# thu-wangz17/HermNet

Hardware: AMD Instinct MI355X
Metric: atom-steps/sec (energy+forces) on 10k-atom 3-element cell; HBM GB/s vs roofline (higher is better)
Workload: dtype f32; 1 GPU; configs[1]: 10000-atom 3-element fcc alloy (Al/Ni/Cu), HVNet rc=5.0 hidden=128 num_rbf=128 layers=5, E=431340 directed edges, energy+forces per step; config=c2, atoms_total=10000, atoms_owned_rank0=10000, halo_atoms_rank0=0, edges_rank0=431340, tuned_gemm_table=False, gemm_tuning_in_warmup=False, parallelism=1 GPU

## Files before the change

### hermnet_amd/csrc/message_bwd_cl.hip

```cpp
#include <hip/hip_runtime.h>
#include <stdint.h>
#include <type_traits>
#include "../../include/hermnet_hip.h"
#include "hermnet_math.h"
#include "message_bwd_cl.h"

namespace {

typedef float hn_f2 __attribute__((ext_vector_type(2)));
typedef unsigned hn_u2 __attribute__((ext_vector_type(2)));
typedef __attribute__((address_space(4))) const float hn_cfloat;
typedef __attribute__((address_space(4))) const int hn_cint;

constexpr int kRec = HN_EDGE_TABLE_FLOATS;

#ifndef HN_NT_TABLE
#define HN_NT_TABLE 1
#endif
__device__ __forceinline__ float fwd_envelope_val(float u, int kind, int p) {
#pragma clang fp contract(off)
  if (kind != 0 || !(u < 1.0f)) return hn_envelope(u, kind, p).val;
  const float up = hn_powi(u, p - 1) * u;
  const float w = 1.0f - u;
  const float fp = (float)p;
  const float inner = __builtin_fmaf(0.5f * fp * (fp + 1.0f), w, fp);
  const float q = 1.0f + w * inner;
  return __builtin_fmaf(-q, up, 1.0f);
}
__global__ __launch_bounds__(256) void edge_table_kernel(const float4* __restrict__ edge, const int* __restrict__ csc_pos,
                                                         int E, const float* __restrict__ offset, int R, float inv_rc,
                                                         float coeff, int env_kind, int env_p,
                                                         float* __restrict__ table, const int* __restrict__ csc_end,
                                                         float* __restrict__ fwd_taps, int csc_blocks) {
  constexpr int kLd = kRec + 4;
  __shared__ __align__(16) float stage[4][64 * kLd];
  const int lane = threadIdx.x & 63, wave = threadIdx.x >> 6;
  if ((int)blockIdx.x >= csc_blocks) {
    constexpr int kF = HN_FWD_TAPS_FLOATS, kLdF = kF + 4;
    const int e0 = (((int)blockIdx.x - csc_blocks) * 4 + wave) * 64;
    if (e0 >= E) return;
    const float u = edge[min(e0 + lane, E - 1)].w * inv_rc;
    const float env_val = fwd_envelope_val(u, env_kind, env_p);
    const int lo = hn_window_lo(u, R);
    float t[kF];
#pragma unroll
    for (int m = 0; m < HN_TAPS; ++m) {
      int k = lo + m;
      k = k < 0 ? 0 : (k >= R ? R - 1 : k);
      const float diff = u - offset[k];
      t[m] = __expf(coeff * (diff * diff));
    }
    t[12] = env_val;
    t[13] = __int_as_float(lo + HN_PAD);
    t[14] = t[15] = 0.f;
    float* st = stage[wave];
#pragma unroll
    for (int w = 0; w < kF / 4; ++w)
      *reinterpret_cast<float4*>(st + lane * kLdF + 4 * w) = make_float4(t[4 * w], t[4 * w + 1], t[4 * w + 2], t[4 * w + 3]);
    const int nrec = min(64, E - e0);
    float4* out = reinterpret_cast<float4*>(fwd_taps + (size_t)e0 * kF);
#pragma unroll
    for (int j = 0; j < kF / 4; ++j) {
      const int idx = j * 64 + lane, r = idx / (kF / 4), w = idx % (kF / 4);
      if (r < nrec) out[idx] = *reinterpret_cast<const float4*>(st + r * kLdF + 4 * w);
    }
    return;
  }
  const int q0 = (blockIdx.x * 4 + wave) * 64;
  if (q0 >= E) return;
  const int q = q0 + lane;
  const int n_csc = csc_end[0];
  float rec[kRec];
#pragma unroll
  for (int w = 0; w < kRec; ++w) rec[w] = 0.f;
  rec[24] = __int_as_float(HN_PAD);
  rec[25] = __int_as_float(HN_PAD);
  if (q < n_csc) {
    const float4 g = edge[csc_pos[q]];
    const float d_next = edge[csc_pos[min(q + 1, n_csc - 1)]].w;
    const float u = g.w * inv_rc;
    const HnEnv env = hn_envelope(u, env_kind, env_p);
    const int lo = hn_window_lo(u, R);
    const float c0 = inv_rc * env.der, c1 = inv_rc * env.val * 2.0f * coeff;
#pragma unroll
    for (int m = 0; m < HN_TAPS; ++m) {
      int k = lo + m;
      k = k < 0 ? 0 : (k >= R ? R - 1 : k);
      const float diff = u - offset[k];
      const float gm = __expf(coeff * (diff * diff));
      rec[2 * m] = env.val * gm;
      rec[2 * m + 1] = c0 * gm + c1 * (gm * diff);
    }
    rec[24] = __int_as_float(lo + HN_PAD);
    rec[25] = __int_as_float(hn_window_lo(d_next * inv_rc, R) + HN_PAD);
    rec[28] = g.x; rec[29] = g.y; rec[30] = g.z;
    rec[31] = __builtin_amdgcn_rcpf(g.w);
  }
  float* st = stage[wave];
#pragma unroll
  for (int w = 0; w < kRec / 4; ++w)
    *reinterpret_cast<float4*>(st + lane * kLd + 4 * w) = make_float4(rec[4 * w], rec[4 * w + 1], rec[4 * w + 2], rec[4 * w + 3]);
  const int nrec = min(64, E - q0);
  float4* out = reinterpret_cast<float4*>(table + (size_t)q0 * kRec);
#pragma unroll
  for (int j = 0; j < kRec / 4; ++j) {
    const int idx = j * 64 + lane, r = idx / (kRec / 4), w = idx % (kRec / 4);
    if (r < nrec) {
#if HN_NT_TABLE
      typedef float f4v __attribute__((ext_vector_type(4)));
      __builtin_nontemporal_store(*reinterpret_cast<const f4v*>(st + r * kLd + 4 * w), reinterpret_cast<f4v*>(out + idx));
#else
      out[idx] = *reinterpret_cast<const float4*>(st + r * kLd + 4 * w);
#endif
    }
  }
  if (q0 + nrec == E && lane < kRec / 4)
    out[(size_t)nrec * (kRec / 4) + lane] = *reinterpret_cast<const float4*>(st + (nrec - 1) * kLd + 4 * lane);
}

template <int CTRL>
__device__ __forceinline__ float dpp_mov(float v) {
  return __int_as_float(__builtin_amdgcn_update_dpp(0, __float_as_int(v), CTRL, 0xF, 0xF, false));
}

__device__ __forceinline__ float pair_fold(float e0, float e1) {
  const hn_u2 s = __builtin_amdgcn_permlane32_swap(__float_as_uint(e0), __float_as_uint(e1), false, false);
  return __uint_as_float(s[0]) + __uint_as_float(s[1]);
}
__device__ __forceinline__ float quad_total(float u, float w) {
  const hn_u2 s = __builtin_amdgcn_permlane16_swap(__float_as_uint(u), __float_as_uint(w), false, false);
  float v = __uint_as_float(s[0]) + __uint_as_float(s[1]);
  v += dpp_mov<0xB1>(v);
  v += dpp_mov<0x4E>(v);
  v += dpp_mov<0x141>(v);
  v += dpp_mov<0x140>(v);
  return v;
}

typedef float hn_f4 __attribute__((ext_vector_type(4)));
__device__ __forceinline__ void lds_issue4(unsigned addr, hn_f4 (&w)[4]) {
  asm volatile(
      "ds_read_b128 %0, %4\n\t"
      "ds_read_b128 %1, %4 offset:1024\n\t"
      "ds_read_b128 %2, %4 offset:2048\n\t"
      "ds_read_b128 %3, %4 offset:3072"
      : "=&v"(w[0]), "=&v"(w[1]), "=&v"(w[2]), "=&v"(w[3])
      : "v"(addr)
      : "memory");
}
__device__ __forceinline__ void lds_wait_all(hn_f4 (&wa)[4], hn_f4 (&wb)[4], hn_f4 (&wc)[4]) {
  asm volatile("s_waitcnt lgkmcnt(0)"
               : "+v"(wa[0]), "+v"(wa[1]), "+v"(wa[2]), "+v"(wa[3]), "+v"(wb[0]), "+v"(wb[1]), "+v"(wb[2]), "+v"(wb[3]),
                 "+v"(wc[0]), "+v"(wc[1]), "+v"(wc[2]), "+v"(wc[3])
               :: "memory");
}
static_assert(HN_CB * 16 == 1024 && HN_TAPS == 12, "the tap reader hard-codes the 1 KiB row pitch and 3 x 4 taps");

typedef __amdgpu_buffer_rsrc_t hn_rsrc;
__device__ __forceinline__ float buf_load(hn_rsrc r, unsigned voff, unsigned soff) {
  return __uint_as_float(__builtin_amdgcn_raw_buffer_load_b32(r, voff, soff, 0));
}

__device__ __forceinline__ void buf_store(hn_rsrc r, unsigned voff, unsigned soff, float v) {
  __builtin_amdgcn_raw_buffer_store_b32(__float_as_uint(v), r, voff, soff, 0);
}
#ifndef HN_NT_MSG
#define HN_NT_MSG 1
#endif
__device__ __forceinline__ float buf_load_once(hn_rsrc r, unsigned voff, unsigned soff) {
  return __uint_as_float(__builtin_amdgcn_raw_buffer_load_b32(r, voff, soff, HN_NT_MSG ? 2 : 0));
}
__device__ __forceinline__ hn_rsrc row_rsrc(unsigned long long base, unsigned row_offset_elems, int H) {
  return __builtin_amdgcn_make_buffer_rsrc((void*)(base + (unsigned long long)row_offset_elems * 4ull), 0, 3 * H * 4, 0x00020000);
}
__device__ __forceinline__ unsigned long long uniform_addr(const void* p) {
  const unsigned long long v = (unsigned long long)p;
  const unsigned lo = (unsigned)__builtin_amdgcn_readfirstlane((int)(unsigned)v);
  const unsigned hi = (unsigned)__builtin_amdgcn_readfirstlane((int)(unsigned)(v >> 32));
  return ((unsigned long long)hi << 32) | lo;
}

struct EdgeIn {
  float gx1, g0, g1, g2;
};

#ifndef HN_KO_BWD
#define HN_KO_BWD 0
#endif
template <bool HAS_VEC, bool WIN, bool NEED_GXH>
__device__ __forceinline__ void message_scatter_bwd_cl_body(const HnBwdClArgs& a) {
  static_assert(NEED_GXH || !HAS_VEC, "rows with a vec part always hand gradients down");
  extern __shared__ __align__(16) float4 tile[];
  const int tile_rows = WIN ? a.win_rows : a.R + 2 * HN_PAD + 1;
  const int tile_base = WIN ? a.win_base : 0;

  int bx = blockIdx.x, by = blockIdx.y, bz = blockIdx.z;
  if (a.xcd_remap) {
    const int total = gridDim.x * gridDim.y * gridDim.z, per = total >> 3;
    int L = bx + gridDim.x * (by + gridDim.y * bz);
    if (L < per * 8) {
      L = (L & 7) * per + (L >> 3);
      bx = L % gridDim.x; by = (L / gridDim.x) % gridDim.y; bz = L / (gridDim.x * gridDim.y);
    }
  }
  const int t = __builtin_amdgcn_readfirstlane(bz);
  const int cb = __builtin_amdgcn_readfirstlane(by);
  int r0, r1;
  if (a.num_ranges > 0) {
    int c = __builtin_amdgcn_readfirstlane(bx);
    r0 = r1 = 0;
    bool found = false;
    for (int k = 0; k < a.num_ranges && !found; ++k) {
      const int lo = a.src_ranges[2 * k], hi = a.src_ranges[2 * k + 1];
      const int nb = hi > lo ? (hi - lo + a.rows_per_block - 1) / a.rows_per_block : 0;
      if (c < nb) { r0 = lo + c * a.rows_per_block; r1 = min(r0 + a.rows_per_block, hi); found = true; }
      c -= nb;
    }
    if (!found) return;
    r0 = __builtin_amdgcn_readfirstlane(r0);
    r1 = __builtin_amdgcn_readfirstlane(r1);
  } else {
    r0 = __builtin_amdgcn_readfirstlane(bx) * a.rows_per_block;
    r1 = min(r0 + a.rows_per_block, a.Nsrc);
  }
  const int lane = threadIdx.x & 63;
  const int wave = __builtin_amdgcn_readfirstlane(threadIdx.x >> 6);
  const int nwaves = blockDim.x >> 6;
  const int H = a.H;
  const unsigned c = (unsigned)(cb * HN_CB + lane);
  const float inv_sqrt3h = 0.57735026918962576f * rsqrtf((float)H);
  const float inv_sqrth = rsqrtf((float)H);
  const float inv_sqrt2 = 0.70710678118654752f;
  float4* gedge = a.gedge + (size_t)cb * a.E;
  const int row16 = lane >> 4;
  const unsigned tile_lane = (unsigned)(unsigned long long)((__attribute__((address_space(3))) char*)tile) + (unsigned)lane * 16u;

  const hn_rsrc rs_gx1 = __builtin_amdgcn_make_buffer_rsrc(const_cast<float*>(a.gx1), 0, (int)((size_t)a.N * H * 4), 0x00020000);
  const hn_rsrc rs_gvec1 = __builtin_amdgcn_make_buffer_rsrc(const_cast<float*>(a.gvec1), 0, (int)((size_t)a.N * 3 * H * 4), 0x00020000);
  const unsigned c4 = c * 4u;

  for (int idx = threadIdx.x; idx < tile_rows * HN_CB; idx += blockDim.x) {
    const int k = idx / HN_CB + tile_base - HN_PAD, ch = idx % HN_CB;
    float4 v = make_float4(0.f, 0.f, 0.f, 0.f);
    if (k >= 0 && k < a.R) {
      const float* w = a.wt + ((size_t)(t * a.R + k) * 3 * H + cb * HN_CB + ch);
      v = make_float4(w[0], w[H], w[2 * H], 0.f);
    }
    tile[idx] = v;
  }

  const unsigned long long xh_t = uniform_addr(a.xh + (size_t)t * a.Nsrc * 3 * H);
  const unsigned long long gxh_t = NEED_GXH ? uniform_addr(a.gxh + (size_t)t * a.Nsrc * 3 * H) : 0ull;
  const unsigned long long gvec_t = HAS_VEC ? uniform_addr(a.gvec + (size_t)t * a.Nsrc * 3 * H) : 0ull;
  const unsigned long long vec_a = HAS_VEC ? uniform_addr(a.vec) : 0ull;
  const int* rowptr_t = a.csc_rowptr + (size_t)t * a.Nsrc;
  const float* brow = a.brbf + (size_t)t * 3 * H;
  const float bs = brow[c], ba = (brow + H)[c], bb = (brow + 2 * H)[c];
  float xbs = 0.f, xba = 0.f, xbb = 0.f;
  if (a.xh_bias) {
    const float* xrow = a.xh_bias + (size_t)t * 3 * H;
    xbs = xrow[c]; xba = (xrow + H)[c]; xbb = (xrow + 2 * H)[c];
  }

  const int E0 = rowptr_t[r0], E1 = rowptr_t[r1];
  const long span = (long)E1 - E0;
  const int es = E0 + (int)(span * wave / nwaves);
  const int ee = (wave + 1 == nwaves) ? E1 + 1 : E0 + (int)(span * (wave + 1) / nwaves);
  int ra = r0, rb = r0;
  for (int q = r0; q < r1; q += 64) {
    const int rq = q + lane;
    const int start = rq < r1 ? rowptr_t[rq] : 0x7fffffff;
    ra += __popcll(__ballot(start < es));
    rb += __popcll(__ballot(start < ee));
  }
  __syncthreads();

  if (ra < rb) {
    const hn_cint* rowptr_c = (const hn_cint*)uniform_addr(rowptr_t);
    int row = ra;
    const int e_begin = rowptr_c[ra];
    const int e_end = rowptr_c[rb];
    int row_end = rowptr_c[row + 1];
    int row_end2 = rowptr_c[min(row + 2, a.Nsrc)];

    float xs = 0.f, xa = 0.f, xas = 0.f, xb = 0.f, vj0 = 0.f, vj1 = 0.f, vj2 = 0.f;
    float raw_s = 0.f, raw_a = 0.f, raw_b = 0.f, raw_v0 = 0.f, raw_v1 = 0.f, raw_v2 = 0.f;
    bool fresh = false;
    float gs = 0.f, ga = 0.f, gb = 0.f, gv0 = 0.f, gv1 = 0.f, gv2 = 0.f;
    const unsigned h4 = (unsigned)(H * 4);
    auto row_request = [&](int r) {
      const unsigned ro = (unsigned)__builtin_amdgcn_readfirstlane(r * (3 * H));
      const hn_rsrc xr = row_rsrc(xh_t, ro, H);
      raw_s = buf_load_once(xr, c4, 0); raw_a = buf_load_once(xr, c4, h4); raw_b = buf_load_once(xr, c4, 2 * h4);
      if (HAS_VEC) {
        const hn_rsrc vr = row_rsrc(vec_a, ro, H);
        raw_v0 = buf_load_once(vr, c4, 0); raw_v1 = buf_load_once(vr, c4, h4); raw_v2 = buf_load_once(vr, c4, 2 * h4);
      }
      gs = 0.f; ga = 0.f; gb = 0.f; gv0 = 0.f; gv1 = 0.f; gv2 = 0.f;
      fresh = true;
    };
    auto row_scale = [&]() {
      xs = (raw_s + xbs) * inv_sqrt2; xa = raw_a + xba; xb = (raw_b + xbb) * inv_sqrth;
      xas = xa * inv_sqrt3h;
      if (HAS_VEC) { vj0 = raw_v0 * inv_sqrt3h; vj1 = raw_v1 * inv_sqrt3h; vj2 = raw_v2 * inv_sqrt3h; }
      fresh = false;
    };
    auto row_epilogue = [&](int r) {
      if constexpr (!NEED_GXH) return;
      const unsigned ro = (unsigned)__builtin_amdgcn_readfirstlane(r * (3 * H));
      const hn_rsrc go = row_rsrc(gxh_t, ro, H);
      if constexpr (WIN) {
        float o0 = gs * inv_sqrt2, o1 = ga, o2 = gb * inv_sqrth;
        if (a.win_accumulate) { o0 += buf_load(go, c4, 0); o1 += buf_load(go, c4, h4); o2 += buf_load(go, c4, 2 * h4); }
        buf_store(go, c4, 0, o0); buf_store(go, c4, h4, o1); buf_store(go, c4, 2 * h4, o2);
      } else {
        buf_store(go, c4, 0, gs * inv_sqrt2); buf_store(go, c4, h4, ga); buf_store(go, c4, 2 * h4, gb * inv_sqrth);
      }
      if (HAS_VEC) {
        const hn_rsrc gvo = row_rsrc(gvec_t, ro, H);
        if constexpr (WIN) {
          if (a.win_accumulate) { gv0 += buf_load(gvo, c4, 0); gv1 += buf_load(gvo, c4, h4); gv2 += buf_load(gvo, c4, 2 * h4); }
        }
        buf_store(gvo, c4, 0, gv0); buf_store(gvo, c4, h4, gv1); buf_store(gvo, c4, 2 * h4, gv2);
      }
    };
    auto win_row = [&](int prow) { return min(max(prow - a.win_base, 0), a.win_rows - HN_TAPS); };
    auto win_owns = [&](int prow) { return (prow >= a.win_lo && prow < a.win_hi) ? 1u : 0u; };
    unsigned own_cur = 1u;
    unsigned own_mask = 0u;
    row_request(row);

    float rec[24];
    float tl0[5], tl1[5];
    hn_f4 wA[4], wB[4], wC[4];
    const hn_cfloat* rp = (const hn_cfloat*)(a.table + (size_t)e_begin * kRec);
    auto load_record = [&](float (&tl)[5]) {
#pragma unroll
      for (int w = 0; w < 24; ++w) rec[w] = rp[w];
      tl[0] = rp[25];
#pragma unroll
      for (int w = 0; w < 4; ++w) tl[1 + w] = rp[28 + w];
    };
    auto issue_weights = [&](unsigned waddr) {
      lds_issue4(waddr, wA);
      lds_issue4(waddr + 4 * (HN_CB * 16), wB);
      lds_issue4(waddr + 8 * (HN_CB * 16), wC);
    };
    if (e_begin < e_end) {
      load_record(tl0);
      if constexpr (WIN) {
        const int prow0 = __float_as_int(rp[24]);
        own_cur = win_owns(prow0);
        issue_weights((unsigned)win_row(prow0) * (HN_CB * 16) + tile_lane);
      } else {
        issue_weights((unsigned)__float_as_int(rp[24]) * (HN_CB * 16) + tile_lane);
      }
    }
    for (int base = e_begin; base < e_end; base += 64) {
      const int cnt = min(64, e_end - base);
      const unsigned my_off = lane < cnt ? (unsigned)a.csc_tgt[base + lane] * (unsigned)(H * 4) : 0u;
      const int my_pos = lane < cnt ? a.csc_pos[base + lane] : 0;

      auto load_edge = [&](int k) {
        EdgeIn in;
        const unsigned so = (unsigned)__builtin_amdgcn_readlane((int)my_off, k);
        in.gx1 = buf_load(rs_gx1, c4, so);
        in.g0 = buf_load(rs_gvec1, c4, 3u * so);
        in.g1 = buf_load(rs_gvec1, c4, 3u * so + h4);
        in.g2 = buf_load(rs_gvec1, c4, 3u * so + 2 * h4);
        return in;
      };

      EdgeIn in0 = load_edge(0), in1 = in0;
      float px[2], py[2], pz[2];
      float ux[2], uy[2], uz[2];
      auto edge_body = [&](auto J, int k) {
        constexpr int j = decltype(J)::value;
        while (base + k >= row_end) {
          row_epilogue(row);
          ++row;
          row_end = row_end2;
          row_end2 = rowptr_c[min(row + 2, a.Nsrc)];
          row_request(row);
        }
        const int kn = j == 3 ? min(k + 1, 63) : k + 1;
        if (j & 1) in0 = load_edge(kn); else in1 = load_edge(kn);
        const EdgeIn& cur = (j & 1) ? in1 : in0;
        float (&tl)[5] = (j & 1) ? tl1 : tl0;
        hn_f2 Ss = {0.f, 0.f}, Sa = {0.f, 0.f}, Sb = {0.f, 0.f};
        auto taps4 = [&](int m0, const hn_f4 (&w)[4]) {
#pragma unroll
          for (int q = 0; q < 4; ++q) {
            const hn_f2 g = {rec[2 * (m0 + q)], rec[2 * (m0 + q) + 1]};
            Ss = __builtin_elementwise_fma(g, hn_f2{w[q].x, w[q].x}, Ss);
            if (HAS_VEC) Sa = __builtin_elementwise_fma(g, hn_f2{w[q].y, w[q].y}, Sa);
            Sb = __builtin_elementwise_fma(g, hn_f2{w[q].z, w[q].z}, Sb);
          }
        };
        lds_wait_all(wA, wB, wC);
#if HN_KO_BWD == 1
        Ss = hn_f2{rec[0] * wA[0].x, rec[1]}; Sa = hn_f2{rec[2] * wB[0].y, rec[3]}; Sb = hn_f2{rec[4] * wC[0].z, rec[5]};
#else
        taps4(0, wA);
        taps4(4, wB);
        taps4(8, wC);
#endif
        unsigned waddr_next;
        float own = 1.0f;
        if constexpr (WIN) {
          const int prow_next = __float_as_int(tl[0]);
          waddr_next = (unsigned)win_row(prow_next) * (HN_CB * 16) + tile_lane;
          own = own_cur ? 1.0f : 0.0f;
          own_mask = j == 0 ? own_cur : (own_mask | (own_cur << j));
          own_cur = win_owns(prow_next);
        } else {
          waddr_next = (unsigned)__float_as_int(tl[0]) * (HN_CB * 16) + tile_lane;
        }
        __builtin_amdgcn_sched_barrier(0);
        asm volatile("" : "+v"(Ss), "+v"(Sa), "+v"(Sb));
        rp += kRec;
        if (j & 1) load_record(tl0); else load_record(tl1);
        issue_weights(waddr_next);
        __builtin_amdgcn_sched_barrier(0);
        if (fresh) row_scale();
#if HN_KO_BWD == 2
        {
          gs += Ss.x + Ss.y + cur.gx1; ga += Sa.x + Sa.y + cur.g0; gb += Sb.x + Sb.y + cur.g1 + cur.g2;
          px[j & 1] = gs; py[j & 1] = ga; pz[j & 1] = gb;
          return;
        }
#endif
        const float rx = tl[1], ry = tl[2], rz = tl[3], invd = tl[4];
        const float gx1 = WIN ? cur.gx1 * own : cur.gx1, g0 = WIN ? cur.g0 * own : cur.g0;
        const float g1 = WIN ? cur.g1 * own : cur.g1, g2 = WIN ? cur.g2 * own : cur.g2;
        const float rs = Ss.x + bs;
        if (NEED_GXH) gs = fmaf(gx1, rs, gs);
        float pdv = gx1 * xs * Ss.y;
        if (HAS_VEC) {
          const float ra_ = Sa.x + ba;
          const float A = fmaf(g0, vj0, fmaf(g1, vj1, g2 * vj2));
          ga = fmaf(A, ra_, ga);
          const float w = xas * ra_;
          gv0 = fmaf(g0, w, gv0); gv1 = fmaf(g1, w, gv1); gv2 = fmaf(g2, w, gv2);
          pdv = fmaf(A * xa, Sa.y, pdv);
        }
        const float rb_ = Sb.x + bb;
        const float B = fmaf(rx, g0, fmaf(ry, g1, rz * g2));
        if (NEED_GXH) gb = fmaf(B, rb_, gb);
        pdv = fmaf(B * xb, Sb.y, pdv);
        const float qi = xb * rb_ * invd;
        const float tpar = fmaf(-B, qi, pdv);
        px[j & 1] = fmaf(tpar, rx, g0 * qi); py[j & 1] = fmaf(tpar, ry, g1 * qi); pz[j & 1] = fmaf(tpar, rz, g2 * qi);
      };
      auto fold = [&](int h) {
        ux[h] = pair_fold(px[0], px[1]); uy[h] = pair_fold(py[0], py[1]); uz[h] = pair_fold(pz[0], pz[1]);
      };
      auto group_store = [&](int k4) {
        const float sx = quad_total(ux[0], ux[1]), sy = quad_total(uy[0], uy[1]), sz = quad_total(uz[0], uz[1]);
        const int je = (row16 == 0) ? 0 : (row16 == 1 ? 2 : (row16 == 2 ? 1 : 3));
        const int p0 = __builtin_amdgcn_readlane(my_pos, k4), p1 = __builtin_amdgcn_readlane(my_pos, min(k4 + 1, cnt - 1));
        const int p2 = __builtin_amdgcn_readlane(my_pos, min(k4 + 2, cnt - 1)), p3 = __builtin_amdgcn_readlane(my_pos, min(k4 + 3, cnt - 1));
        const int pw = (row16 == 0) ? p0 : (row16 == 1 ? p2 : (row16 == 2 ? p1 : p3));
        if constexpr (WIN) {
          if ((lane & 15) == 0 && k4 + je < cnt && ((own_mask >> je) & 1u)) gedge[pw] = make_float4(sx, sy, sz, 0.f);
        } else {
#if HN_NT_MSG
          if ((lane & 15) == 0 && k4 + je < cnt)
            __builtin_nontemporal_store(hn_f4{sx, sy, sz, 0.f}, reinterpret_cast<hn_f4*>(&gedge[pw]));
#else
          if ((lane & 15) == 0 && k4 + je < cnt) gedge[pw] = make_float4(sx, sy, sz, 0.f);
#endif
        }
      };
      using I0 = std::integral_constant<int, 0>; using I1 = std::integral_constant<int, 1>;
      using I2 = std::integral_constant<int, 2>; using I3 = std::integral_constant<int, 3>;
      int k4 = 0;
      for (; k4 + 4 <= cnt; k4 += 4) {
        edge_body(I0{}, k4); edge_body(I1{}, k4 + 1); fold(0);
        edge_body(I2{}, k4 + 2); edge_body(I3{}, k4 + 3); fold(1);
        group_store(k4);
      }
      if (k4 < cnt) {
        px[1] = 0.f; py[1] = 0.f; pz[1] = 0.f;
        edge_body(I0{}, k4);
        if (k4 + 1 < cnt) edge_body(I1{}, k4 + 1);
        fold(0);
        px[0] = 0.f; py[0] = 0.f; pz[0] = 0.f; px[1] = 0.f; py[1] = 0.f; pz[1] = 0.f;
        if (k4 + 2 < cnt) edge_body(I2{}, k4 + 2);
        fold(1);
        group_store(k4);
      }
    }
    for (;;) {
      row_epilogue(row);
      if (++row >= rb) break;
      gs = 0.f; ga = 0.f; gb = 0.f; gv0 = 0.f; gv1 = 0.f; gv2 = 0.f;
    }
  }
}

template <bool HAS_VEC, bool WIN>
__global__ __launch_bounds__(1024, 4) void message_scatter_bwd_cl_kernel(HnBwdClArgs a) {
  message_scatter_bwd_cl_body<HAS_VEC, WIN, true>(a);
}
template <bool WIN>
__global__ __launch_bounds__(1024, 4) void message_edge_bwd_cl_kernel(HnBwdClArgs a) {
  message_scatter_bwd_cl_body<false, WIN, false>(a);
}

__global__ __launch_bounds__(256) void message_bwd_finish_kernel(const float4* __restrict__ part, int T, long n4_vec,
                                                                 const float4* __restrict__ gvec1,
                                                                 const float4* __restrict__ gx1,
                                                                 const int* __restrict__ type_rowptr, int identity,
                                                                 int H, float4* __restrict__ gvec, float4* __restrict__ gx,
                                                                 long n4_x, const int* __restrict__ ranges, int num_ranges) {
  const long i = (long)blockIdx.x * blockDim.x + threadIdx.x;
  const int identity_rows = identity ? type_rowptr[T] : 0;
  if (num_ranges > 0) {
    bool vin = false, xin = false;
    const long rv = i / (3 * H / 4), rx = i / (H / 4);
    for (int k = 0; k < num_ranges; ++k) {
      const int lo = ranges[2 * k], hi = ranges[2 * k + 1];
      vin |= rv >= lo && rv < hi;
      xin |= rx >= lo && rx < hi;
    }
    if (!vin) n4_vec = 0;
    if (!xin) n4_x = 0;
  }
  if (part && i < n4_vec) {
    float4 acc = part[i];
    for (int t = 1; t < T; ++t) {
      const float4 v = part[(long)t * n4_vec + i];
      acc.x += v.x; acc.y += v.y; acc.z += v.z; acc.w += v.w;
    }
    if (i / (3 * H / 4) < identity_rows) {
      const float4 v = gvec1[i];
      acc.x += v.x; acc.y += v.y; acc.z += v.z; acc.w += v.w;
    }
    gvec[i] = acc;
  }
  if (i < n4_x) {
    float4 v = make_float4(0.f, 0.f, 0.f, 0.f);
    if (i / (H / 4) < identity_rows) {
      const float4 g = gx1[i];
      const float s = 0.70710678118654752f;
      v = make_float4(g.x * s, g.y * s, g.z * s, g.w * s);
    }
    gx[i] = v;
  }
}

int num_cus() {
  static int n = 0;
  if (n == 0) {
    int dev = 0, v = 0;
    if (hipGetDevice(&dev) == hipSuccess &&
        hipDeviceGetAttribute(&v, hipDeviceAttributeMultiprocessorCount, dev) == hipSuccess && v > 0) n = v;
    else n = 256;
  }
  return n;
}

}

size_t hn_bwd_cl_lds_bytes(int R) {
  return (size_t)(R + 2 * HN_PAD + 1) * HN_CB * sizeof(float4);
}

int hn_bwd_cl_launch(HnBwdClArgs a, bool has_vec, bool need_gxh, int rows_override, const int* ranges_host, hipStream_t s) {
  if (!need_gxh && (has_vec || a.gx != nullptr)) return HN_ERR_BAD_ARG;
  constexpr int kMaxRows = 160;
  const int rows_all = a.R + 2 * HN_PAD + 1;
  const bool windowed = rows_all > kMaxRows;
  const int split = (rows_all - HN_PAD + 1) / 2;
  if (windowed && (split + HN_PAD > kMaxRows || rows_all - split > kMaxRows)) return HN_ERR_LDS;
  const size_t lds = windowed ? (size_t)(split + HN_PAD > rows_all - split ? split + HN_PAD : rows_all - split) * HN_CB * sizeof(float4)
                              : hn_bwd_cl_lds_bytes(a.R);
  typedef void (*kern_t)(HnBwdClArgs);
  kern_t k = windowed ? (has_vec ? message_scatter_bwd_cl_kernel<true, true> : message_scatter_bwd_cl_kernel<false, true>)
                      : (has_vec ? message_scatter_bwd_cl_kernel<true, false> : message_scatter_bwd_cl_kernel<false, false>);
  if (!need_gxh) k = windowed ? message_edge_bwd_cl_kernel<true> : message_edge_bwd_cl_kernel<false>;
  static bool done[6] = {false, false, false, false, false, false};
  const int which = need_gxh ? (windowed ? 2 : 0) + (has_vec ? 1 : 0) : (windowed ? 5 : 4);
  if (!done[which]) {
    if (hipFuncSetAttribute(reinterpret_cast<const void*>(k), hipFuncAttributeMaxDynamicSharedMemorySize,
                            kMaxRows * HN_CB * (int)sizeof(float4)) != hipSuccess)
      return HN_ERR_LDS;
    done[which] = true;
  }
  const int ncb = a.H / HN_CB;
  int rpb = rows_override;
  long rows = a.Nsrc;
  if (a.num_ranges > 0) {
    if (!ranges_host || !a.src_ranges || a.num_ranges > 16) return HN_ERR_BAD_ARG;
    rows = 0;
    for (int k = 0; k < a.num_ranges; ++k) {
      const int lo = ranges_host[2 * k], hi = ranges_host[2 * k + 1];
      if (lo < 0 || hi > a.Nsrc || (k > 0 && lo < ranges_host[2 * k - 1])) return HN_ERR_BAD_ARG;
      if (hi > lo) rows += hi - lo;
    }
    if (rows == 0) return HN_OK;
  }
  if (rpb <= 0) {
    const long work = rows * ncb * a.T;
    const int cus = num_cus();
    long rounds = (work + (long)cus * 128) / ((long)cus * 256);
    if (rounds < 1) rounds = 1;
    long wgs_per_tc = cus * rounds / ((long)ncb * a.T);
    if (wgs_per_tc < 1) wgs_per_tc = 1;
    rpb = (int)((rows + wgs_per_tc - 1) / wgs_per_tc);
    if (rpb < 16) rpb = 16;
    if (a.num_ranges > 0) {
      for (int it = 0; it < 64; ++it) {
        long c = 0;
        for (int k = 0; k < a.num_ranges; ++k) {
          const int lo = ranges_host[2 * k], hi = ranges_host[2 * k + 1];
          if (hi > lo) c += (hi - lo + rpb - 1) / rpb;
        }
        if (c <= wgs_per_tc) break;
        rpb += (rpb + 31) / 32;
      }
    }
  }
  a.rows_per_block = rpb;
  long chunks = (a.Nsrc + rpb - 1) / rpb;
  if (a.num_ranges > 0) {
    chunks = 0;
    for (int k = 0; k < a.num_ranges; ++k) {
      const int lo = ranges_host[2 * k], hi = ranges_host[2 * k + 1];
      if (hi > lo) chunks += (hi - lo + rpb - 1) / rpb;
    }
  }
  dim3 grid((unsigned)chunks, (unsigned)ncb, (unsigned)a.T);
  if (!windowed) {
    hipLaunchKernelGGL(k, grid, dim3(1024), lds, s, a);
  } else {
    a.win_base = 0; a.win_rows = split + HN_PAD; a.win_lo = 0; a.win_hi = split; a.win_accumulate = 0;
    hipLaunchKernelGGL(k, grid, dim3(1024), lds, s, a);
    a.win_base = split; a.win_rows = rows_all - split; a.win_lo = split; a.win_hi = 0x7fffffff; a.win_accumulate = 1;
    hipLaunchKernelGGL(k, grid, dim3(1024), lds, s, a);
  }
  if (a.gx == nullptr) return hipGetLastError() == hipSuccess ? HN_OK : HN_ERR_LAUNCH;
  const long n4v = has_vec ? (long)a.Nsrc * 3 * a.H / 4 : 0, n4x = (long)a.Nsrc * a.H / 4;
  const long n4 = n4v > n4x ? n4v : n4x;
  hipLaunchKernelGGL(message_bwd_finish_kernel, dim3((unsigned)((n4 + 255) / 256)), dim3(256), 0, s,
                     has_vec ? reinterpret_cast<const float4*>(a.gvec) : nullptr, a.T, n4v,
                     reinterpret_cast<const float4*>(a.gvec1), reinterpret_cast<const float4*>(a.gx1),
                     a.type_rowptr, a.identity, a.H, reinterpret_cast<float4*>(a.gvec_out),
                     reinterpret_cast<float4*>(a.gx), n4x, a.src_ranges, a.num_ranges);
  return hipGetLastError() == hipSuccess ? HN_OK : HN_ERR_LAUNCH;
}

extern "C" int hermnet_edge_radial_tables(const hn_graph* g, const hn_rbf_desc* rbf, const float* edge, float* table,
                                          float* fwd_taps, void* stream) {
  if (!g || !rbf || rbf->num_rbf < 2 || g->num_edges < 0) return HN_ERR_BAD_ARG;
  const int num_edges = g->num_edges;
  if (num_edges == 0) return HN_OK;
  if (!edge || !table || !rbf->offset || !g->csc_pos || !g->csc_rowptr) return HN_ERR_BAD_ARG;
  const int csc_blocks = (num_edges + 255) / 256;
  hipLaunchKernelGGL(edge_table_kernel, dim3(fwd_taps ? 2 * csc_blocks : csc_blocks), dim3(256), 0, (hipStream_t)stream,
                     reinterpret_cast<const float4*>(edge), g->csc_pos, num_edges, rbf->offset, rbf->num_rbf, rbf->inv_rc,
                     rbf->coeff, rbf->env_kind, rbf->env_p, table,
                     g->csc_rowptr + (size_t)g->num_rel * (size_t)(g->num_src > 0 ? g->num_src : g->num_nodes), fwd_taps,
                     csc_blocks);
  return hipGetLastError() == hipSuccess ? HN_OK : HN_ERR_LAUNCH;
}

extern "C" int hermnet_edge_radial_table(const hn_graph* g, const hn_rbf_desc* rbf, const float* edge, float* table,
                                         void* stream) {
  return hermnet_edge_radial_tables(g, rbf, edge, table, nullptr, stream);
}
```

Before: 3.827 million atom-steps/s.

## Balance backward message scatter work across types by edge count

```diff
diff --git a/hermnet_amd/csrc/message_bwd_cl.hip b/hermnet_amd/csrc/message_bwd_cl.hip
--- a/hermnet_amd/csrc/message_bwd_cl.hip
+++ b/hermnet_amd/csrc/message_bwd_cl.hip
@@ -184,6 +184,27 @@
   float gx1, g0, g1, g2;
 };
 
+__device__ __forceinline__ void lower_bound_pair(const int* __restrict__ p, int n, int ka, int kb, int lane, int& ra, int& rb) {
+  int loa = 0, hia = n, lob = 0, hib = n;
+  while (hia > loa || hib > lob) {
+    const int na = hia - loa, nb = hib - lob;
+    const int sa = (na + 63) >> 6, sb = (nb + 63) >> 6;
+    const int va = na > 0 ? p[loa + min((lane + 1) * sa, na) - 1] : 0x7fffffff;
+    const int vb = nb > 0 ? p[lob + min((lane + 1) * sb, nb) - 1] : 0x7fffffff;
+    const int ca = __popcll(__ballot(va < ka)), cb = __popcll(__ballot(vb < kb));
+    if (na > 0) {
+      if (ca < 64) hia = loa + min((ca + 1) * sa, na) - 1;
+      loa += min(ca * sa, na);
+    }
+    if (nb > 0) {
+      if (cb < 64) hib = lob + min((cb + 1) * sb, nb) - 1;
+      lob += min(cb * sb, nb);
+    }
+  }
+  ra = __builtin_amdgcn_readfirstlane(loa);
+  rb = __builtin_amdgcn_readfirstlane(lob);
+}
+
 #ifndef HN_KO_BWD
 #define HN_KO_BWD 0
 #endif
@@ -203,18 +224,90 @@
       bx = L % gridDim.x; by = (L / gridDim.x) % gridDim.y; bz = L / (gridDim.x * gridDim.y);
     }
   }
-  const int t = __builtin_amdgcn_readfirstlane(bz);
+  int t = __builtin_amdgcn_readfirstlane(bz);
   const int cb = __builtin_amdgcn_readfirstlane(by);
-  int r0, r1;
-  if (a.num_ranges > 0) {
-    int c = __builtin_amdgcn_readfirstlane(bx);
+  const int lane = threadIdx.x & 63;
+  const int wave = __builtin_amdgcn_readfirstlane(threadIdx.x >> 6);
+  const int nwaves = blockDim.x >> 6;
+  const int H = a.H;
+  const unsigned c = (unsigned)(cb * HN_CB + lane);
+  const bool balanced = a.rows_per_block <= 0;
+  int r0 = 0, r1 = 0;
+  int es = 0, ee = 0;
+  if (balanced) {
+    const unsigned wc = gridDim.x, w = (unsigned)__builtin_amdgcn_readfirstlane(bx);
+    const int T = a.T;
+    const int lo_e = lane < T ? a.csc_rowptr[(size_t)lane * a.Nsrc] : 0;
+    const int hi_e = lane < T ? a.csc_rowptr[(size_t)(lane + 1) * a.Nsrc] : 0;
+    const unsigned e = (unsigned)(hi_e - lo_e);
+    unsigned etot = 0;
+    for (int j = 0; j < T; ++j) etot += (unsigned)__builtin_amdgcn_readlane((int)e, j);
+    if constexpr (NEED_GXH) {
+      unsigned long long empty = (WIN && a.win_accumulate) ? 0ull : __ballot(lane < T && e == 0u);
+      while (empty) {
+        const int tz = __ffsll(empty) - 1;
+        empty &= empty - 1;
+        for (unsigned r = w * nwaves + wave; r < (unsigned)a.Nsrc; r += wc * nwaves) {
+          float* g = a.gxh + ((size_t)tz * a.Nsrc + r) * 3 * H;
+          g[c] = 0.f; (g + H)[c] = 0.f; (g + 2 * H)[c] = 0.f;
+          if (HAS_VEC) {
+            float* gv = a.gvec + ((size_t)tz * a.Nsrc + r) * 3 * H;
+            gv[c] = 0.f; (gv + H)[c] = 0.f; (gv + 2 * H)[c] = 0.f;
+          }
+        }
+      }
+    }
+    if (etot == 0u) return;
+    const unsigned long long prod = (unsigned long long)e * wc;
+    const unsigned q = (unsigned)(prod / etot), rem = (unsigned)(prod - (unsigned long long)q * etot);
+    unsigned sumq = 0, rank = 0;
+    for (int j = 0; j < T; ++j) {
+      sumq += (unsigned)__builtin_amdgcn_readlane((int)q, j);
+      const unsigned rj = (unsigned)__builtin_amdgcn_readlane((int)rem, j);
+      rank += (rj > rem || (rj == rem && j < lane)) ? 1u : 0u;
+    }
+    unsigned n = (lane < T && rank < wc - sumq) ? q + 1u : q;
+    for (;;) {
+      const unsigned long long need = __ballot(lane < T && e > 0u && n == 0u);
+      if (!need) break;
+      const int tz = __ffsll(need) - 1;
+      unsigned best = 0;
+      int donor = 0;
+      for (int j = 0; j < T; ++j) {
+        const unsigned nj = (unsigned)__builtin_amdgcn_readlane((int)n, j);
+        if (nj > best) { best = nj; donor = j; }
+      }
+      if (lane == tz) n = 1u;
+      if (lane == donor) n -= 1u;
+    }
+    unsigned start = 0;
+    for (int j = 0; j < T; ++j) {
+      const unsigned nj = (unsigned)__builtin_amdgcn_readlane((int)n, j);
+      start += j < lane ? nj : 0u;
+    }
+    const unsigned long long mine = __ballot(lane < T && w >= start && w < start + n);
+    if (!mine) return;
+    t = __builtin_amdgcn_readfirstlane(__ffsll(mine) - 1);
+    const unsigned idx = w - (unsigned)__builtin_amdgcn_readlane((int)start, t);
+    const unsigned long long shares = (unsigned long long)(unsigned)__builtin_amdgcn_readlane((int)n, t) * nwaves;
+    const unsigned long long et = (unsigned)__builtin_amdgcn_readlane((int)e, t);
+    const int E0 = __builtin_amdgcn_readlane(lo_e, t);
+    const unsigned long long s0 = (unsigned long long)idx * nwaves;
+    auto cut = [&](unsigned long long s) {
+      return s == shares ? E0 + (int)et + 1 : E0 + (int)(et * s / shares);
+    };
+    if (cut(s0) == cut(s0 + nwaves)) return;
+    es = __builtin_amdgcn_readfirstlane(cut(s0 + wave));
+    ee = __builtin_amdgcn_readfirstlane(cut(s0 + wave + 1));
+  } else if (a.num_ranges > 0) {
+    int chunk = __builtin_amdgcn_readfirstlane(bx);
     r0 = r1 = 0;
     bool found = false;
     for (int k = 0; k < a.num_ranges && !found; ++k) {
       const int lo = a.src_ranges[2 * k], hi = a.src_ranges[2 * k + 1];
       const int nb = hi > lo ? (hi - lo + a.rows_per_block - 1) / a.rows_per_block : 0;
-      if (c < nb) { r0 = lo + c * a.rows_per_block; r1 = min(r0 + a.rows_per_block, hi); found = true; }
-      c -= nb;
+      if (chunk < nb) { r0 = lo + chunk * a.rows_per_block; r1 = min(r0 + a.rows_per_block, hi); found = true; }
+      chunk -= nb;
     }
     if (!found) return;
     r0 = __builtin_amdgcn_readfirstlane(r0);
@@ -223,11 +316,6 @@
     r0 = __builtin_amdgcn_readfirstlane(bx) * a.rows_per_block;
     r1 = min(r0 + a.rows_per_block, a.Nsrc);
   }
-  const int lane = threadIdx.x & 63;
-  const int wave = __builtin_amdgcn_readfirstlane(threadIdx.x >> 6);
-  const int nwaves = blockDim.x >> 6;
-  const int H = a.H;
-  const unsigned c = (unsigned)(cb * HN_CB + lane);
   const float inv_sqrt3h = 0.57735026918962576f * rsqrtf((float)H);
   const float inv_sqrth = rsqrtf((float)H);
   const float inv_sqrt2 = 0.70710678118654752f;
@@ -262,16 +350,21 @@
     xbs = xrow[c]; xba = (xrow + H)[c]; xbb = (xrow + 2 * H)[c];
   }
 
-  const int E0 = rowptr_t[r0], E1 = rowptr_t[r1];
-  const long span = (long)E1 - E0;
-  const int es = E0 + (int)(span * wave / nwaves);
-  const int ee = (wave + 1 == nwaves) ? E1 + 1 : E0 + (int)(span * (wave + 1) / nwaves);
-  int ra = r0, rb = r0;
-  for (int q = r0; q < r1; q += 64) {
-    const int rq = q + lane;
-    const int start = rq < r1 ? rowptr_t[rq] : 0x7fffffff;
-    ra += __popcll(__ballot(start < es));
-    rb += __popcll(__ballot(start < ee));
+  int ra, rb;
+  if (balanced) {
+    lower_bound_pair(rowptr_t, a.Nsrc, es, ee, lane, ra, rb);
+  } else {
+    const int E0 = rowptr_t[r0], E1 = rowptr_t[r1];
+    const long span = (long)E1 - E0;
+    es = E0 + (int)(span * wave / nwaves);
+    ee = (wave + 1 == nwaves) ? E1 + 1 : E0 + (int)(span * (wave + 1) / nwaves);
+    ra = r0; rb = r0;
+    for (int q = r0; q < r1; q += 64) {
+      const int rq = q + lane;
+      const int start = rq < r1 ? rowptr_t[rq] : 0x7fffffff;
+      ra += __popcll(__ballot(start < es));
+      rb += __popcll(__ballot(start < ee));
+    }
   }
   __syncthreads();
 
@@ -591,6 +684,7 @@
   const int ncb = a.H / HN_CB;
   int rpb = rows_override;
   long rows = a.Nsrc;
+  const bool balanced = rows_override <= 0 && a.num_ranges == 0 && a.T <= 64;
   if (a.num_ranges > 0) {
     if (!ranges_host || !a.src_ranges || a.num_ranges > 16) return HN_ERR_BAD_ARG;
     rows = 0;
@@ -601,37 +695,44 @@
     }
     if (rows == 0) return HN_OK;
   }
-  if (rpb <= 0) {
-    const long work = rows * ncb * a.T;
-    const int cus = num_cus();
-    long rounds = (work + (long)cus * 128) / ((long)cus * 256);
-    if (rounds < 1) rounds = 1;
-    long wgs_per_tc = cus * rounds / ((long)ncb * a.T);
-    if (wgs_per_tc < 1) wgs_per_tc = 1;
-    rpb = (int)((rows + wgs_per_tc - 1) / wgs_per_tc);
-    if (rpb < 16) rpb = 16;
+  const int cus = num_cus();
+  long rounds = (rows * ncb * a.T + (long)cus * 128) / ((long)cus * 256);
+  if (rounds < 1) rounds = 1;
+  dim3 grid;
+  if (balanced) {
+    long wgs_per_cb = cus * rounds / ncb;
+    if (wgs_per_cb < a.T) wgs_per_cb = a.T;
+    a.rows_per_block = 0;
+    grid = dim3((unsigned)wgs_per_cb, (unsigned)ncb, 1);
+  } else {
+    if (rpb <= 0) {
+      long wgs_per_tc = cus * rounds / ((long)ncb * a.T);
+      if (wgs_per_tc < 1) wgs_per_tc = 1;
+      rpb = (int)((rows + wgs_per_tc - 1) / wgs_per_tc);
+      if (rpb < 16) rpb = 16;
+      if (a.num_ranges > 0) {
+        for (int it = 0; it < 64; ++it) {
+          long c = 0;
+          for (int k = 0; k < a.num_ranges; ++k) {
+            const int lo = ranges_host[2 * k], hi = ranges_host[2 * k + 1];
+            if (hi > lo) c += (hi - lo + rpb - 1) / rpb;
+          }
+          if (c <= wgs_per_tc) break;
+          rpb += (rpb + 31) / 32;
+        }
+      }
+    }
+    a.rows_per_block = rpb;
+    long chunks = (a.Nsrc + rpb - 1) / rpb;
     if (a.num_ranges > 0) {
-      for (int it = 0; it < 64; ++it) {
-        long c = 0;
-        for (int k = 0; k < a.num_ranges; ++k) {
-          const int lo = ranges_host[2 * k], hi = ranges_host[2 * k + 1];
-          if (hi > lo) c += (hi - lo + rpb - 1) / rpb;
-        }
-        if (c <= wgs_per_tc) break;
-        rpb += (rpb + 31) / 32;
-      }
-    }
-  }
-  a.rows_per_block = rpb;
-  long chunks = (a.Nsrc + rpb - 1) / rpb;
-  if (a.num_ranges > 0) {
-    chunks = 0;
-    for (int k = 0; k < a.num_ranges; ++k) {
-      const int lo = ranges_host[2 * k], hi = ranges_host[2 * k + 1];
-      if (hi > lo) chunks += (hi - lo + rpb - 1) / rpb;
-    }
-  }
-  dim3 grid((unsigned)chunks, (unsigned)ncb, (unsigned)a.T);
+      chunks = 0;
+      for (int k = 0; k < a.num_ranges; ++k) {
+        const int lo = ranges_host[2 * k], hi = ranges_host[2 * k + 1];
+        if (hi > lo) chunks += (hi - lo + rpb - 1) / rpb;
+      }
+    }
+    grid = dim3((unsigned)chunks, (unsigned)ncb, (unsigned)a.T);
+  }
   if (!windowed) {
     hipLaunchKernelGGL(k, grid, dim3(1024), lds, s, a);
   } else {
```

Result: no change. 3.859 million atom-steps/s (median of 6 runs) (+0.8%).
